# TravisWheelerLab/BATH

Hardware: AMD Instinct MI355X
Metric: DP Gcells/s + residues/s through bathsearch pipeline at 1/2/4/8 MI355X (higher is better)
Workload: dtype u8/i16 integer scores (SSV: exact binary16), f32 Forward

## Files before the change

### bath_amd/csrc/bath_kernels.hpp

```cpp
#pragma once
#include <climits>
#include <hip/hip_runtime.h>

#include <cstdint>

#include "bath_hip.h"

namespace bath {

typedef short s16x2 __attribute__((ext_vector_type(2)));

template <int CTRL, int ROW_MASK = 0xf>
__device__ __forceinline__ int dpp_i(int v, int old) { return __builtin_amdgcn_update_dpp(old, v, CTRL, ROW_MASK, 0xf, false); }
__device__ __forceinline__ int wave_shr1_i32(int v, int fill) { return dpp_i<0x138>(v, fill); }
__device__ __forceinline__ float wave_shr1_f32(float v, float fill) {
  return __builtin_bit_cast(float, __builtin_amdgcn_update_dpp(__builtin_bit_cast(int, fill), __builtin_bit_cast(int, v), 0x138, 0xf, 0xf, false));
}
__device__ __forceinline__ float wave_max_f32(float v) {
  const int ninf = (int)0xff800000;
#define BATH_FMAX_STEP(CTRL, MASK) v = fmaxf(v, __builtin_bit_cast(float, __builtin_amdgcn_update_dpp(ninf, __builtin_bit_cast(int, v), CTRL, MASK, 0xf, false)));
  BATH_FMAX_STEP(0x111, 0xf) BATH_FMAX_STEP(0x112, 0xf) BATH_FMAX_STEP(0x114, 0xf) BATH_FMAX_STEP(0x118, 0xf) BATH_FMAX_STEP(0x142, 0xa) BATH_FMAX_STEP(0x143, 0xc)
#undef BATH_FMAX_STEP
  return __builtin_bit_cast(float, __builtin_amdgcn_readlane(__builtin_bit_cast(int, v), 63));
}
__device__ __forceinline__ int wave_max_i32(int v) {
  v = max(v, dpp_i<0x111>(v, INT_MIN)); v = max(v, dpp_i<0x112>(v, INT_MIN)); v = max(v, dpp_i<0x114>(v, INT_MIN));
  v = max(v, dpp_i<0x118>(v, INT_MIN)); v = max(v, dpp_i<0x142, 0xa>(v, INT_MIN)); v = max(v, dpp_i<0x143, 0xc>(v, INT_MIN));
  return __builtin_amdgcn_readlane(v, 63);
}
__device__ __forceinline__ int wave_min_i32(int v) {
  v = min(v, dpp_i<0x111>(v, INT_MAX)); v = min(v, dpp_i<0x112>(v, INT_MAX)); v = min(v, dpp_i<0x114>(v, INT_MAX));
  v = min(v, dpp_i<0x118>(v, INT_MAX)); v = min(v, dpp_i<0x142, 0xa>(v, INT_MAX)); v = min(v, dpp_i<0x143, 0xc>(v, INT_MAX));
  return __builtin_amdgcn_readlane(v, 63);
}
__device__ __forceinline__ float wave_sum_f32(float v) {
#ifdef BATH_SUM_BPERMUTE
#pragma unroll
  for (int d = 32; d >= 1; d >>= 1) v += __shfl_xor(v, d, 64);
// ... 78 lines not shown
  return (grank == 0) ? kSsvBeginPair : far;
}
template <int G>
__device__ __forceinline__ int ssv_group_max(s16x2 xE) {
  typedef _Float16 h16x2 __attribute__((ext_vector_type(2)));
  const h16x2 h = __builtin_bit_cast(h16x2, xE);
  int v = (int)(fmaxf((float)h.x, (float)h.y) * 2048.0f) - 128;
#pragma unroll
  for (int d = SsvGroups<G>::TPW; d < 64; d <<= 1) v = max(v, __shfl_xor(v, d, 64));
  return v;
}

struct MsvConsts {
  int tbm, tec, base, bias;
  float scale_b;
};

__device__ __forceinline__ int ssv_classify(int v, int tjb, const MsvConsts &c, float *sc) {
  if (tjb + c.tbm + c.tec + c.bias >= 127) return BATH_ENORESULT;
  unsigned xE = (v >= -1 - c.bias) ? 255u : (unsigned)(v + 256);
  if ((int)xE >= 255 - c.bias) {
    *sc = INFINITY;
    return (c.base - tjb - c.tbm < 128) ? BATH_ENORESULT : BATH_ERANGE;
  }
  xE = (xE + (unsigned)(c.base - tjb - c.tbm) - 128u) & 0xffffu;
  if ((int)xE >= 255 - c.bias) { *sc = INFINITY; return BATH_ERANGE; }
  unsigned xJ = (xE - (unsigned)c.tec) & 0xffffu;
  if ((int)xJ > c.base) return BATH_ENORESULT;
  float r = ((float)((int)xJ - tjb) - (float)c.base);
  r /= c.scale_b;
  r = (float)((double)r - 3.0);
  *sc = r;
  return BATH_OK;
}

struct WindowRec { int32_t cand, n, k, length; float score; };

__device__ __forceinline__ float bias_forward(const uint8_t *s, int L, int M, const float *e , float p1) {
  const float L1 = (float)M / 8.0f;
  const float t00 = p1, t01 = 1.0f - p1, t10 = 1.0f / (L1 + 1.0f), t11 = L1 / (L1 + 1.0f);
  float logsc = 0.0f;
  if (L <= 0) return logsc;
  int x = min((int)s[0], 28);
  float d0 = e[2 * x] * 0.999f, d1 = e[2 * x + 1] * 0.001f;
  float mx = fmaxf(fmaxf(d0, 0.0f), d1);
  d0 /= mx; d1 /= mx;
  logsc += (float)log((double)mx);
  auto step = [&](int xx) {
    float n0 = 0.0f + d0 * t00; n0 = n0 + d1 * t10; n0 *= e[2 * xx];
    float n1 = 0.0f + d0 * t01; n1 = n1 + d1 * t11; n1 *= e[2 * xx + 1];
    mx = fmaxf(fmaxf(n0, 0.0f), n1);
    d0 = n0 / mx; d1 = n1 / mx;
    logsc += (float)log((double)mx);
  };
  int i = 1;
  uint32_t wnext = (i + 4 <= L) ? *reinterpret_cast<const uint32_t *>(s + i) : 0u;
  for (; i + 4 <= L; i += 4) {
    const uint32_t w = wnext;
    if (i + 8 <= L) wnext = *reinterpret_cast<const uint32_t *>(s + i + 4);
#pragma unroll
    for (int j = 0; j < 4; j++) step(min((int)((w >> (8 * j)) & 0xffu), 28));
  }
  for (; i < L; i++) step(min((int)s[i], 28));
  float end = 0.0f + d0 * 1.0f; end = end + d1 * 1.0f;
  logsc += (float)log((double)end);
  return logsc;
// ... 4 lines not shown
```

### bath_amd/csrc/bath_launch.hpp

```cpp
#pragma once
#include <utility>

#include "bath_common.hpp"

#define BATH_SSV_SHAPES(X)                                                                                   \
  X(16, 1) X(20, 1) X(24, 1) X(28, 1) X(32, 1) X(36, 1) X(40, 1) X(44, 1) X(48, 1) X(52, 1) X(56, 1) X(60, 1) X(64, 1)     \
  X(68, 1) X(72, 1) X(76, 1) X(80, 1) X(84, 1) X(88, 1) X(92, 1) X(96, 1) X(100, 1) X(104, 1) X(108, 1) X(112, 1)           \
  X(128, 1) X(144, 1) X(160, 1) X(176, 1) X(192, 1) X(208, 1)                                                \
  X(40, 2) X(48, 2) X(56, 2) X(64, 2) X(72, 2) X(76, 2)                                                     \
  X(112, 2) X(128, 2) X(144, 2) X(160, 2) X(176, 2) X(192, 2) X(208, 2)                                      \
  X(112, 4) X(128, 4) X(144, 4) X(160, 4) X(176, 4) X(192, 4) X(208, 4)                                      \
  X(112, 8) X(128, 8) X(144, 8) X(160, 8) X(176, 8) X(192, 8) X(208, 8)

namespace bath {

struct Cand {
  int64_t *window;  int32_t *sf;
  int32_t *startj;  int32_t *len;
  int16_t *v;
  int64_t *off;
  int32_t *msv_status, *vit_status, *fwd_status, *stage, *flags;
  float *usc, *nullsc, *filtersc, *vfsc, *fwdsc;
  double *P;
  int32_t *kminmax;
};

int build_orf_records(bath_hip_ctx *ctx, const Cand &cand, int nc, int64_t window_offset, bath_orf_result **d_out, int64_t *n_out);

struct VitWindowArgs {
  double invP_vit, invP_msv;
  const float *d_filtersc;
  const uint8_t *d_ssv_scores;
  void *d_wins;
  int *d_win_count;
  int win_cap;
  int32_t *d_kminmax;
};

int launch_ssv_lane(bath_hip_ctx *ctx, const bath_hip_oprofile *om, SeqView v, const int32_t *d_order, int16_t *d_v);
int launch_ssv_classify(bath_hip_ctx *ctx, const bath_hip_oprofile *om, int64_t n, const int32_t *d_len, const int16_t *d_v, float *d_sc, int32_t *d_status);
int launch_msv_wave(bath_hip_ctx *ctx, const bath_hip_oprofile *om, SeqView v, const int32_t *d_todo, int64_t ntodo, float *d_sc, int32_t *d_status, const int *ntodo_dev, bool lane_ok = true);
int launch_msv_lane(bath_hip_ctx *ctx, const bath_hip_oprofile *om, SeqView v, const int32_t *d_todo, int64_t ntodo, float *d_sc, int32_t *d_status, const int *ntodo_dev);
int launch_vit_wave(bath_hip_ctx *ctx, const bath_hip_oprofile *om, SeqView v, const int32_t *d_todo, int64_t ntodo, float *d_sc, int32_t *d_status,
                    const VitWindowArgs *wa, const int *ntodo_dev);
int launch_fwd_wave(bath_hip_ctx *ctx, const bath_hip_oprofile *om, SeqView v, const int32_t *d_todo, int64_t ntodo, float *d_sc, int32_t *d_status, const int *ntodo_dev,
                    float *d_xmx = nullptr, const int64_t *d_xmx_off = nullptr, float *d_dp = nullptr, const int64_t *d_dp_off = nullptr, int unihit = 0,
                    const int32_t *d_cfg_len = nullptr);
int launch_bwd_wave(bath_hip_ctx *ctx, const bath_hip_oprofile *om, SeqView v, int64_t n, const float *d_fwd_xmx, const int64_t *d_xmx_off,
                    float *d_sc, int32_t *d_status, float *d_bck_xmx, float *d_dp = nullptr, const int64_t *d_dp_off = nullptr, int unihit = 0);
int launch_bias_lane(bath_hip_ctx *ctx, const bath_hip_oprofile *om, SeqView v, const float *d_eo, int eo_stride, const int32_t *d_todo, int64_t ntodo,
                     float *d_nullsc, float *d_filtersc);

int vit_lane_supported(const bath_hip_oprofile *om);
int launch_len_sort(bath_hip_ctx *ctx, const int32_t *d_todo, const int *d_ntodo, const int32_t *d_len, int *d_bins, int32_t *d_sorted);
int launch_vit_lane(bath_hip_ctx *ctx, const bath_hip_oprofile *om, SeqView v, const int32_t *d_todo, int64_t ntodo, const int *ntodo_dev,
                    float *d_sc, int32_t *d_status, const VitWindowArgs *wa, const int *skip_dev = nullptr);
const int *len_sort_count_longer(const int *d_bins, int T);
int64_t lane_min_nt();
const char *vit_lane_kernel_name(const bath_hip_oprofile *om);
int launch_vit_sorted(bath_hip_ctx *ctx, const bath_hip_oprofile *om, SeqView v, const int32_t *d_todo, int64_t cap, const int *d_ntodo, const int32_t *d_len,
                      int *d_bins, int32_t *d_sorted, float *d_sc, int32_t *d_status, const VitWindowArgs *wa, const std::function<int(hipStream_t)> &beside);
struct MsvConsts;
MsvConsts msv_consts(const bath_hip_oprofile *om);

int pipeline_filters_survivors(bath_hip_ctx *ctx, const bath_hip_oprofile *om, const bath_hip_seqs *dna, const bath_pipeline_params *prm,
                               bath_pipeline_stats *stats, std::vector<PipelineSurvivor> *out, const uint8_t **d_pool);

struct FsWinDev {
  int64_t src_off;
  int64_t dst_off;
  int32_t seq_n, start, len, strand, kmin, kmax;
};
int fs_gather_view(bath_hip_ctx *ctx, const bath_hip_seqs *dna, std::vector<FsWinDev> &regs, const uint8_t *d_comp, bath_hip_seqs *view, const FsWinDev **d_desc_out);

struct WindowRec;
// ... 92 lines not shown
```

### bath_amd/csrc/bath_msv_lane.hip

```cpp
#include "bath_common.hpp"
#include "bath_kernels.hpp"
#include "bath_launch.hpp"

using namespace bath;

namespace bath {

__device__ __forceinline__ s16x2 msv_pkmax(s16x2 a, s16x2 b) {
  s16x2 r;
  asm("v_pk_max_f16 %0, %1, %2" : "=v"(r) : "v"(a), "v"(b));
  return r;
}

template <int NR>
__global__ __launch_bounds__(256, NR <= 76 ? 4 : 1) void msv_lane_kernel(SeqView sq, const int16_t *__restrict__ cost_tab , int row_bytes,
                                                                        const uint8_t *__restrict__ tjb_tab, MsvConsts c,
                                                                        const int32_t *__restrict__ todo, int64_t ntodo, const int *__restrict__ ntodo_dev,
                                                                        float *__restrict__ sc, int32_t *__restrict__ status) {
  extern __shared__ __attribute__((aligned(16))) char lds[];
  {
    const int n32 = kSsvRows * row_bytes / 4;
    const uint32_t *src = reinterpret_cast<const uint32_t *>(cost_tab);
    uint32_t *dst = reinterpret_cast<uint32_t *>(lds);
    for (int i = threadIdx.x; i < n32; i += blockDim.x) dst[i] = src[i];
  }
  __syncthreads();
  if (ntodo_dev) ntodo = *ntodo_dev;
  const int lane = threadIdx.x & 63;
  const int64_t nwaves = ((int64_t)gridDim.x * blockDim.x) >> 6;
  typedef _Float16 h16x2 __attribute__((ext_vector_type(2)));
  for (int64_t w = ((int64_t)blockIdx.x * blockDim.x + threadIdx.x) >> 6; w * 64 < ntodo; w += nwaves) {
    const int64_t job = w * 64 + lane;
    const bool live = job < ntodo;
    const int64_t sid = live ? (todo ? (int64_t)todo[job] : job) : 0;
    const int L = live ? sq.len[sid] : 0;
    const uint8_t *s = sq.data + sq.off[sid];
    const int Lw = wave_max_i32(L);
    const int tjb = tjb_tab[L];
    const int tjbm = (uint8_t)((int8_t)tjb + (int8_t)c.tbm);
    s16x2 reg[NR];
    const s16x2 zero = {0, 0};
#pragma unroll
    for (int r = 0; r < NR; r++) reg[r] = zero;
    int xJ = 0, xB = satu8(c.base - tjbm);
    bool overflow = false;
    uint2 res = make_uint2(0u, 0u);
    for (int i = 0; i < Lw; i++) {
      if ((i & 7) == 0) {
        if (i + 8 <= L) __builtin_memcpy(&res, s + i, 8);
        else {
          res = make_uint2(0u, 0u);
          for (int j = 0; j < 8 && i + j < L; j++) {
            const unsigned b = s[i + j];
            if (j < 4) res.x |= b << (8 * j); else res.y |= b << (8 * (j - 4));
          }
        }
      }
      const unsigned byte = (((i & 4) ? res.y : res.x) >> (8 * (i & 3))) & 0xffu;
      const int x = (i < L) ? min((int)byte, kKp - 1) : kRowReset;
      const ssv_i4 *row = reinterpret_cast<const ssv_i4 *>(lds + (size_t)x * row_bytes);
      const h16x2 bh = {(_Float16)((float)xB * (1.0f / 2048.0f)), (_Float16)((float)xB * (1.0f / 2048.0f))};
      const s16x2 xBv = __builtin_bit_cast(s16x2, bh);
      const s16x2 wrap = __builtin_bit_cast(s16x2, __builtin_amdgcn_alignbit(__builtin_bit_cast(unsigned, reg[NR - 1]), 0u, 16));
      s16x2 xE = zero, xE2 = zero;
#pragma unroll
      for (int g = NR / 4 - 1; g >= 0; g--) {
        const ssv_i4 inc = row[g];
        const int r = 4 * g;
        const s16x2 v3 = ssv_add(msv_pkmax(reg[r + 2], xBv), inc.w);
        const s16x2 v2 = ssv_add(msv_pkmax(reg[r + 1], xBv), inc.z);
        const s16x2 v1 = ssv_add(msv_pkmax(reg[r], xBv), inc.y);
        const s16x2 v0 = ssv_add(msv_pkmax((r > 0) ? reg[r - 1] : wrap, xBv), inc.x);
        reg[r + 3] = v3; reg[r + 2] = v2; reg[r + 1] = v1; reg[r] = v0;
        xE = ssv_max3(xE, v3, v2);
        xE2 = ssv_max3(xE2, v1, v0);
      }
      const h16x2 e1 = __builtin_bit_cast(h16x2, xE), e2 = __builtin_bit_cast(h16x2, xE2);
      int xEi = (int)(fmaxf(fmaxf((float)e1.x, (float)e1.y), fmaxf((float)e2.x, (float)e2.y)) * 2048.0f);
      if (xEi + c.bias >= 255) overflow = true;
      xEi = max(xEi - c.tec, 0);
      xJ = max(xJ, xEi);
      xB = max(max(c.base, xJ) - tjbm, 0);
    }
    if (live) {
      if (overflow) { sc[sid] = INFINITY; status[sid] = BATH_ERANGE; }
      else {
        float r = ((float)(xJ - tjb) - (float)c.base);
        r /= c.scale_b;
        r = (float)((double)r - 3.0);
        sc[sid] = r; status[sid] = BATH_OK;
      }
    }
  }
}

int launch_msv_lane(bath_hip_ctx *ctx, const bath_hip_oprofile *om, SeqView v, const int32_t *d_todo, int64_t ntodo, float *d_sc, int32_t *d_status, const int *ntodo_dev) {
  static const bool off = [] { const char *e = std::getenv("BATH_HIP_MSV_WAVE"); return e && e[0] == '1'; }();
  if (off || om->G != 1 || om->NR > 76 || !om->d_msv) return BATH_ENORESULT;
  if (ntodo == 0) return BATH_OK;
  const size_t shmem = (size_t)kSsvRows * om->ssv_row_bytes;
  const int64_t waves = (ntodo + 63) / 64;
  const int grid = (int)std::max<int64_t>(1, std::min<int64_t>((waves + 3) / 4, (int64_t)ctx->prop.multiProcessorCount * 4));
  bool launched = false;
#define BATH_MSV_CASE(N)                                                                                                               \
  if (!launched && om->NR == N) {                                                                                                      \
    hipLaunchKernelGGL((msv_lane_kernel<N>), dim3(grid), dim3(256), shmem, ctx->stream, v, om->d_msv, om->ssv_row_bytes, om->lt.d_tjb,   \
                       MsvConsts{om->tbm_b, om->tec_b, om->base_b, om->bias_b, om->scale_b}, d_todo, ntodo, ntodo_dev, d_sc, d_status); \
    launched = true;                                                                                                                   \
  }
  BATH_MSV_CASE(16) BATH_MSV_CASE(20) BATH_MSV_CASE(24) BATH_MSV_CASE(28) BATH_MSV_CASE(32) BATH_MSV_CASE(36) BATH_MSV_CASE(40) BATH_MSV_CASE(44)
  BATH_MSV_CASE(48) BATH_MSV_CASE(52) BATH_MSV_CASE(56) BATH_MSV_CASE(60) BATH_MSV_CASE(64) BATH_MSV_CASE(68) BATH_MSV_CASE(72) BATH_MSV_CASE(76)
#undef BATH_MSV_CASE
  if (!launched) return BATH_ENORESULT;
  BATH_HIP_TRY(ctx, hipGetLastError());
  return BATH_OK;
}

}
```

### bath_amd/csrc/bath_pipeline.hip

```cpp
#include <algorithm>
#include <cmath>
#include <cstring>
#include <cstdlib>
#include <map>
#include <thread>

#include "bath_common.hpp"
#include "bath_kernels.hpp"
#include "bath_launch.hpp"
#include "host_model.hpp"

using namespace bath;

namespace bath {

static const double kLog2 = 0.69314718055994529;

enum { FLAG_VIT_RUN = 1, FLAG_HAS_WIN = 2 };

struct Counters {
  int cand_count, todo_msv, todo_vit, todo_ssvb, todo_vit2, todo_fwd, win_count, overflow;
  int todo_lb, pad_;
  unsigned long long n_orfs, orf_res;
  unsigned long long n_past_msv, n_past_bias, n_past_vit, n_past_fwd;
// ... 77 lines not shown
        const int startj = (int32_t)(rec.aa_off - (2 * dna.off[w] + 96 * w + (int64_t)sf * orf_stream_pitch(dna.len[w])));
        const int C = dna.context[w], start_s = sf % 3 + 3 * startj + 1;
        if (sf < 3 ? (start_s + 3 * L - 1 < C) : (dna.len[w] - start_s + 1 < C)) r = (unsigned long long)L;
      }
      if (__ballot(r != 0)) { for (int d = 32; d >= 1; d >>= 1) r += __shfl_xor(r, d, 64); if (lane == 0) atomicAdd(&ctr->res_seen, r); }
    }
    if (live && grank == 0 && v >= (int)emit_thresh[min(L, thresh_max)]) {
      const int sf = (int)((unsigned)rec.len_sf >> 28);
      const int64_t w = rec.w;
      const int64_t stream = 2 * dna.off[w] + 96 * w + (int64_t)sf * orf_stream_pitch(dna.len[w]);
      const int startj = (int32_t)(rec.aa_off - stream);
      bool seen = false;
      if (dna.context) {
        const int C = dna.context[w], start_s = sf % 3 + 3 * startj + 1;
        seen = sf < 3 ? (start_s + 3 * L - 1 < C) : (dna.len[w] - start_s + 1 < C);
      }
      const int slot = seen ? cand_cap + 1 : atomicAdd(&ctr->cand_count, 1);
      if (seen) {
      } else if (slot < cand_cap) {
        cand.window[slot] = w; cand.sf[slot] = sf; cand.startj[slot] = startj; cand.len[slot] = L;
        cand.v[slot] = (int16_t)min(v, 32767); cand.off[slot] = rec.aa_off;
      } else atomicOr(&ctr->overflow, 1);
    }
  }
}

__device__ __forceinline__ double d_gumbel_surv(double x, double mu, double lambda) {
  const double ey = -exp(-lambda * (x - mu));
  if (fabs(ey) < 5e-9) return -ey;
  return 1.0 - exp(ey);
}
__device__ __forceinline__ double d_exp_surv(double x, double mu, double lambda) { return (x < mu) ? 1.0 : exp(-lambda * (x - mu)); }

__global__ void classify_kernel(Cand cand, int cand_cap, Counters *__restrict__ ctr, const uint8_t *__restrict__ tjb_tab, MsvConsts mc,
                                int32_t *__restrict__ todo_msv) {
  const int ncand = min(ctr->cand_count, cand_cap);
  for (int c = blockIdx.x * blockDim.x + threadIdx.x; c < ncand; c += gridDim.x * blockDim.x) {
    float sc = 0.f;
    const int st = ssv_classify(cand.v[c], tjb_tab[cand.len[c]], mc, &sc);
    cand.usc[c] = sc; cand.msv_status[c] = st; cand.stage[c] = 0; cand.flags[c] = 0;
    cand.vfsc[c] = -INFINITY; cand.fwdsc[c] = -INFINITY; cand.vit_status[c] = 0; cand.filtersc[c] = 0.f; cand.P[c] = 1.0;
    cand.kminmax[2 * c] = 1 << 30; cand.kminmax[2 * c + 1] = 0;
    if (st == BATH_ENORESULT) todo_msv[atomicAdd(&ctr->todo_msv, 1)] = c;
  }
}

__global__ void f1_bias_kernel(Cand cand, int cand_cap, Counters *__restrict__ ctr, Params p, const uint8_t *__restrict__ pool, int M,
                               const float *__restrict__ eo, const float *__restrict__ nullsc_tab, const float *__restrict__ p1_tab,
                               const float *__restrict__ lt1_tab, const float *__restrict__ lt2_tab,
                               int32_t *__restrict__ todo_vit, int32_t *__restrict__ todo_ssvb) {
  __shared__ float s_eo[kKp * 2];
  for (int i = threadIdx.x; i < kKp * 2; i += blockDim.x) s_eo[i] = eo[i];
  __syncthreads();
  const int ncand = min(ctr->cand_count, cand_cap);
  for (int c = blockIdx.x * blockDim.x + threadIdx.x; c < ncand; c += gridDim.x * blockDim.x) {
    const int L = cand.len[c];
    const float usc = cand.usc[c];
    const float nullsc = nullsc_tab[L];
    cand.nullsc[c] = nullsc;
    float seqsc = (float)((double)(usc - nullsc) / kLog2);
    double P = d_gumbel_surv(seqsc, p.evparam[0], p.evparam[1]);
    cand.P[c] = P;
    if (P > p.F1) continue;
    atomicAdd(&ctr->n_past_msv, 1ull); atomicAdd(&ctr->pos_past_msv, (unsigned long long)L * 3ull);
    cand.stage[c] = 1;
    float filtersc = nullsc;
    if (p.do_bias) {
      filtersc = bias_forward(pool + cand.off[c], L, M, s_eo, p1_tab[L]);
      filtersc = (filtersc + lt1_tab[L]) + lt2_tab[L];
      seqsc = (float)((double)(usc - filtersc) / kLog2);
      P = d_gumbel_surv(seqsc, p.evparam[0], p.evparam[1]);
      cand.P[c] = P; cand.filtersc[c] = filtersc;
      if (P > p.F1) continue;
    }
    cand.filtersc[c] = filtersc;
    atomicAdd(&ctr->n_past_bias, 1ull); atomicAdd(&ctr->pos_past_bias, (unsigned long long)L * 3ull);
    cand.stage[c] = 2;
    if (P > p.F2) { cand.flags[c] |= FLAG_VIT_RUN; todo_vit[atomicAdd(&ctr->todo_vit, 1)] = c; atomicAdd(&ctr->res_vit, (unsigned long long)L); }
    else todo_ssvb[atomicAdd(&ctr->todo_ssvb, 1)] = c;
  }
}

template <int C>
__global__ __launch_bounds__(256) void ssv_bath_kernel(Cand cand, const Counters *__restrict__ ctr, const int32_t *__restrict__ todo,
                                                       const uint8_t *__restrict__ pool, int M, const uint8_t *__restrict__ rb, int rb_stride,
                                                       const uint8_t *__restrict__ ssv_scores, const uint8_t *__restrict__ tjb_tab,
                                                       const float *__restrict__ nullsc_tab, MsvConsts mc, double invP_f1,
                                                       WindowRec *__restrict__ wins, int win_cap, Counters *__restrict__ ctrw) {
  const int lane = threadIdx.x & 63;
  const int64_t wid = ((int64_t)blockIdx.x * blockDim.x + threadIdx.x) >> 6;
  const int64_t nw = ((int64_t)gridDim.x * blockDim.x) >> 6;
  const int ntodo = ctr->todo_ssvb;
  const int Q = max(2, ((M - 1) / 16) + 1);
  for (int64_t job = wid; job < ntodo; job += nw) {
    const int c = todo[job];
    const int L = cand.len[c];
    const uint8_t *s = pool + cand.off[c];
    const int tjb = tjb_tab[L];
    const float nullsc = nullsc_tab[L];
    const int sc_thresh = (uint8_t)(int)ceil((((double)nullsc + ((double)(float)invP_f1 * kLog2) + 3.0) * (double)mc.scale_b) + mc.base + mc.tec + tjb);
    const int tjbm = (uint8_t)((int8_t)tjb + (int8_t)mc.tbm);
    const int xB = satu8(mc.base - tjbm);
    int kmin = 1 << 30, kmax = 0;
    int dp[C];
#pragma unroll
    for (int k = 0; k < C; k++) dp[k] = 0;
    const int ph = threadIdx.x & 63;
    int rbuf = (ph < L) ? (int)s[ph] : 0, rnext = 0;
    for (int i = 1; i <= L; i++) {
      const int j = (i - 1) & 63;
      if (j == 0) { const int q = i - 1 + 64 + ph; rnext = (q < L) ? (int)s[q] : 0; }
      const int x = min(__builtin_amdgcn_readlane(rbuf, j), kKp - 1);
      if (j == 63) rbuf = rnext;
// ... 444 lines not shown
    SeqView cv{W.pool, W.cand.off, W.cand.len, cap};

    int e = 0;
    BATH_HIP_TRY(ctx, hipEventRecord(ev[e++], ctx->stream));
    if ((st = launch_orf_scan(ctx, dna, tt, prm->min_orf_len, ob, &W.ctr->n_orfs, &W.ctr->orf_res, prm->strands)) != BATH_OK) return st;
    BATH_HIP_TRY(ctx, hipEventRecord(ev[e++], ctx->stream));
    {
      static const int ssv_chunk = [] { const char *e = std::getenv("BATH_HIP_SSV_CHUNK"); return e ? std::atoi(e) : 0; }();
      int blocks = ctx->prop.multiProcessorCount * 4;
      const int ssv_threads = 256;
      const int wpb = ssv_threads / 64;
      if (ssv_chunk > 0) blocks = (int)std::min<int64_t>((max_orfs + (int64_t)wpb * (64 / om->G) * ssv_chunk - 1) / ((int64_t)wpb * (64 / om->G) * ssv_chunk), 1 << 30);
      bool launched = false;
#define BATH_ORF_CASE(N, GG)                                                                                                     \
  if (!launched && NRk == N && om->G == GG) {                                                                                    \
    if (ssv_shmem > 64 * 1024) (void)bath::allow_max_lds((const void *)ssv_orf_kernel<N, GG>); \
    hipLaunchKernelGGL((ssv_orf_kernel<N, GG>), dim3(blocks), dim3(ssv_threads), ssv_shmem, ctx->stream, W.pool, ob.sorted, ob.ntotal,                  \
                       dna->view(), om->d_ssv, om->ssv_row_bytes, d_emit, max_orf, W.cand, W.cand_cap, W.ctr, ssv_chunk);        \
    launched = true;                                                                                                             \
  }
      BATH_SSV_SHAPES(BATH_ORF_CASE)
#undef BATH_ORF_CASE
      if (!launched) { ctx->set_error("SSV kernel: no tile shape for this model length"); return BATH_EINVAL; }
      BATH_HIP_TRY(ctx, hipGetLastError());
    }
    BATH_HIP_TRY(ctx, hipEventRecord(ev[e++], ctx->stream));
    hipStream_t bulk_stream = ctx->stream;
    struct StreamRestore { bath_hip_ctx *c; hipStream_t s; ~StreamRestore() { c->stream = s; } } stream_restore{ctx, bulk_stream};
    if (ctx->tail_stream) {
      BATH_HIP_TRY(ctx, hipStreamWaitEvent(ctx->tail_stream, ev[e - 1], 0));
      ctx->stream = ctx->tail_stream;
    }
    const bool few_cands = dna->total < lane_min_nt(), few_msv = dna->total < 2 * lane_min_nt();
    hipLaunchKernelGGL(classify_kernel, dim3(dec_blocks), dim3(256), 0, ctx->stream, W.cand, W.cand_cap, W.ctr, om->lt.d_tjb, mc, W.todo_msv);
    BATH_HIP_TRY(ctx, hipGetLastError());
    if ((st = launch_msv_wave(ctx, om, cv, W.todo_msv, cap, W.cand.usc, W.cand.msv_status, &W.ctr->todo_msv, !few_msv)) != BATH_OK) return st;
    BATH_HIP_TRY(ctx, hipEventRecord(ev[e++], ctx->stream));
    hipLaunchKernelGGL(f1_bias_kernel, dim3(dec_blocks), dim3(256), 0, ctx->stream, W.cand, W.cand_cap, W.ctr, P, W.pool, M, om->d_bias_eo,
                       om->lt.d_nullsc, om->lt.d_p1, om->lt.d_lt1, om->lt.d_lt2, W.todo_vit, W.todo_ssvb);
    BATH_HIP_TRY(ctx, hipGetLastError());
    BATH_HIP_TRY(ctx, hipEventRecord(ev[e++], ctx->stream));
    wa.d_filtersc = W.cand.filtersc; wa.d_ssv_scores = d_ssvsc; wa.d_wins = W.wins; wa.d_win_count = &W.ctr->win_count; wa.win_cap = W.win_cap;
    wa.d_kminmax = W.cand.kminmax;
    auto launch_ssvb = [&](hipStream_t stream) -> int {
      const int Cc = (M + 63) / 64;
      int Cs = -1;
      for (int opt : {1, 2, 3, 4, 6, 8, 12, 16, 24, 32, 52}) if (Cc <= opt) { Cs = opt; break; }
#define BATH_SSVB_CASE(N)                                                                                                          \
  case N:                                                                                                                          \
    hipLaunchKernelGGL(ssv_bath_kernel<N>, dim3(wave_grid_blocks(ctx) / 4), dim3(256), 0, stream, W.cand, W.ctr, W.todo_ssvb, W.pool, M,      \
                       om->d_rb, om->rb_stride, d_ssvsc, om->lt.d_tjb, om->lt.d_nullsc, mc, invP_f1, W.wins, W.win_cap, W.ctr);    \
    break;
      switch (Cs) {
        BATH_SSVB_CASE(1) BATH_SSVB_CASE(2) BATH_SSVB_CASE(3) BATH_SSVB_CASE(4) BATH_SSVB_CASE(6) BATH_SSVB_CASE(8)
        BATH_SSVB_CASE(12) BATH_SSVB_CASE(16) BATH_SSVB_CASE(24) BATH_SSVB_CASE(32) BATH_SSVB_CASE(52)
        default: ctx->set_error("model too long for the SSV window kernel"); return BATH_EINVAL;
      }
#undef BATH_SSVB_CASE
      return BATH_OK;
    };
    bool ssvb_done = false;
    if (vit_lane_supported(om) && !few_cands) {
      if ((st = launch_vit_sorted(ctx, om, cv, W.todo_vit, cap, &W.ctr->todo_vit, W.cand.len, W.len_bins, W.todo_sorted, W.cand.vfsc, W.cand.vit_status, &wa,
                                  launch_ssvb)) != BATH_OK) return st;
      ssvb_done = true;
    } else if ((st = launch_vit_wave(ctx, om, cv, W.todo_vit, cap, W.cand.vfsc, W.cand.vit_status, &wa, &W.ctr->todo_vit)) != BATH_OK) return st;
    BATH_HIP_TRY(ctx, hipEventRecord(ev[e++], ctx->stream));
    if (!ssvb_done && (st = launch_ssvb(ctx->stream)) != BATH_OK) return st;
    BATH_HIP_TRY(ctx, hipGetLastError());
    BATH_HIP_TRY(ctx, hipEventRecord(ev[e++], ctx->stream));
    hipLaunchKernelGGL(post_vit_kernel, dim3(dec_blocks), dim3(256), 0, ctx->stream, W.cand, W.cand_cap, W.ctr, P, W.todo_msv , W.todo_fwd);
    if (P.do_bias) {
      DevBuf &b_compo = ctx->scratch[36];
      BATH_HIP_TRY(ctx, b_compo.reserve((size_t)20 * 256 * 4 + (size_t)W.cand_cap * 20 * 4 + 256));
// ... 3 lines not shown
      hipLaunchKernelGGL(post_vit_local_kernel, dim3(std::max(1, dec_blocks)), dim3(64), 0, ctx->stream, W.cand, W.ctr, P, W.pool, M, d_bgf, d_compo,
                         om->lt.d_p1, om->lt.d_lt1, om->lt.d_lt2, W.todo_msv, W.todo_vit2, W.todo_fwd);
    }
    BATH_HIP_TRY(ctx, hipGetLastError());
    if ((st = launch_vit_wave(ctx, om, cv, W.todo_vit2, cap, W.cand.vfsc, W.cand.vit_status, nullptr, &W.ctr->todo_vit2)) != BATH_OK) return st;
    hipLaunchKernelGGL(post_vit2_kernel, dim3(64), dim3(256), 0, ctx->stream, W.cand, W.ctr, P, W.todo_vit2, W.todo_fwd);
    BATH_HIP_TRY(ctx, hipGetLastError());
    BATH_HIP_TRY(ctx, hipEventRecord(ev[e++], ctx->stream));
    ctx->fwd_rows_kept = nullptr; ctx->fwd_rows_off = nullptr;
    float *d_keep = nullptr; int64_t *d_keep_off = nullptr;
    if (ctx->keep_fwd_rows) {
      constexpr int64_t kKeepFloats = (int64_t)8 << 20;
      DevBuf &b_rows = ctx->scratch[38], &b_roff = ctx->scratch[39];
      BATH_HIP_TRY(ctx, b_rows.reserve((size_t)kKeepFloats * sizeof(float) + 64)); BATH_HIP_TRY(ctx, b_roff.reserve((size_t)cap * sizeof(int64_t) + 64));
      d_keep = b_rows.as<float>(); d_keep_off = b_roff.as<int64_t>();
      hipLaunchKernelGGL(fwd_keep_offsets_kernel, dim3(1), dim3(64), 0, ctx->stream, W.todo_fwd, &W.ctr->todo_fwd, W.cand.len, d_keep_off, kKeepFloats);
      BATH_HIP_TRY(ctx, hipGetLastError());
    }
    if ((st = launch_fwd_wave(ctx, om, cv, W.todo_fwd, cap, W.cand.fwdsc, W.cand.fwd_status, &W.ctr->todo_fwd, d_keep, d_keep_off)) != BATH_OK) return st;
    if (d_keep) { ctx->fwd_rows_kept = d_keep; ctx->fwd_rows_off = d_keep_off; }
    hipLaunchKernelGGL(final_kernel, dim3(dec_blocks), dim3(256), 0, ctx->stream, W.cand, W.ctr, P, W.todo_fwd);
    BATH_HIP_TRY(ctx, hipGetLastError());
    BATH_HIP_TRY(ctx, hipEventRecord(ev[e++], ctx->stream));

    BATH_HIP_TRY(ctx, hipMemcpyAsync(&hc, W.ctr, sizeof(Counters), hipMemcpyDeviceToHost, ctx->stream));
    BATH_HIP_TRY(ctx, hipStreamSynchronize(ctx->stream));
    if (hc.overflow || hc.cand_count > cap || hc.win_count > W.win_cap) {
      if (attempt >= 4) { ctx->set_error("candidate / window buffers overflowed repeatedly"); return BATH_EMEM; }
      if (hc.overflow || hc.cand_count > cap) cap = std::max<int64_t>(cap * 2, (int64_t)hc.cand_count + 1024);
      if (hc.win_count > W.win_cap) win_need = hc.win_count + hc.win_count / 4 + 1024;
      continue;
    }
    static const char *names[] = {"translate_orfs", "ssv_f1", "classify_msv", "f1_bias", "viterbi_windows", "ssv_windows", "post_vit", "forward_final"};
    static const int64_t launches[] = {4, 1, 2, 1, 4, 1, 3, 2};
    ctx->timings.clear();
    for (int i = 0; i + 1 < e; i++) {
      float ms = 0.f;
      BATH_HIP_TRY(ctx, hipEventElapsedTime(&ms, ev[i], ev[i + 1]));
      ctx->timings.push_back(StageTiming{names[i], ms, launches[i]});
    }
    break;
  }

  if (stats) {
    stats->nres = nres; stats->n_orfs = (int64_t)hc.n_orfs;
    stats->n_past_msv = (int64_t)hc.n_past_msv; stats->n_past_bias = (int64_t)hc.n_past_bias;
    stats->n_past_vit = (int64_t)hc.n_past_vit; stats->n_past_fwd = (int64_t)hc.n_past_fwd;
    stats->pos_past_msv = (int64_t)hc.pos_past_msv; stats->pos_past_bias = (int64_t)hc.pos_past_bias;
    stats->pos_past_vit = (int64_t)hc.pos_past_vit; stats->pos_past_fwd = (int64_t)hc.pos_past_fwd;
    stats->cells_msv = (int64_t)(hc.orf_res - hc.res_seen) * M; stats->cells_vit = (int64_t)hc.res_vit * M; stats->cells_fwd = (int64_t)hc.res_fwd * M;
  }

  if (results) {
    bath_orf_result *d_rec = nullptr;
    int64_t nrec = 0;
    if (dna->n > (int64_t)UINT32_MAX || dna->maxlen / 3 >= (1 << 28)) { ctx->set_error("block too large for the ORF records' sort key (2^32 windows, 805 Mnt per window)"); return BATH_ERANGE; }
    if ((st = build_orf_records(ctx, W.cand, hc.cand_count, dna->is_part ? dna->first_window : 0, &d_rec, &nrec)) != BATH_OK) return st;
    ctx->d_records = d_rec; ctx->n_records = nrec;
    if (!dna->is_part) {
      BATH_HIP_TRY(ctx, ctx->results_pinned.reserve((size_t)std::max<int64_t>(nrec, 1) * sizeof(bath_orf_result)));
      if (nrec > 0) BATH_HIP_TRY(ctx, hipMemcpyAsync(ctx->results_pinned.p, d_rec, (size_t)nrec * sizeof(bath_orf_result), hipMemcpyDeviceToHost, ctx->stream));
      BATH_HIP_TRY(ctx, hipStreamSynchronize(ctx->stream));
      *results = ctx->results_pinned.as<bath_orf_result>();
    } else *results = nullptr;
    if (n_results) *n_results = nrec;
  } else if (n_results) *n_results = (int64_t)hc.n_past_msv;
  if (state) { state->W = W; state->hc = hc; state->d_ssvsc = d_ssvsc; state->d_bgf = d_bgf; state->tt = tt; }
// ... 622 lines not shown
```

Baseline: 197.6 billion.

## Fuse classify, MSV rescoring and F1 bias filter into one stage kernel

Adds a fused msv_stage_kernel. Each thread classifies its candidate, rescores it with the per-lane MSV DP when SSV gave no result, and then runs the F1/bias filter in the same launch. This drops two kernel launches and the todo_msv indirection. In exchange, every block copies the cost table into LDS, and lanes whose candidate needs no rescore sit idle while the rest of the wave runs the MSV loop, so the wave runs as long as its longest rescore. It also launches over cand_cap blocks rather than a bounded grid, which may leave many blocks that exit immediately.

```diff
diff --git a/bath_amd/csrc/bath_kernels.hpp b/bath_amd/csrc/bath_kernels.hpp
--- a/bath_amd/csrc/bath_kernels.hpp
+++ b/bath_amd/csrc/bath_kernels.hpp
@@ -4,6 +4,7 @@
 
 #include <cstdint>
 
+#include "bath_common.hpp"
 #include "bath_hip.h"
 
 namespace bath {
@@ -148,6 +149,67 @@
   r = (float)((double)r - 3.0);
   *sc = r;
   return BATH_OK;
+}
+
+__device__ __forceinline__ s16x2 msv_pkmax(s16x2 a, s16x2 b) {
+  s16x2 r;
+  asm("v_pk_max_f16 %0, %1, %2" : "=v"(r) : "v"(a), "v"(b));
+  return r;
+}
+template <int NR>
+__device__ __forceinline__ int msv_lane_rows(const char *lds, int row_bytes, const uint8_t *s, int L, int Lw, int tjbm, const MsvConsts &c, bool *overflow) {
+  typedef _Float16 h16x2 __attribute__((ext_vector_type(2)));
+  s16x2 reg[NR];
+  const s16x2 zero = {0, 0};
+#pragma unroll
+  for (int r = 0; r < NR; r++) reg[r] = zero;
+  int xJ = 0, xB = satu8(c.base - tjbm);
+  bool over = false;
+  uint2 res = make_uint2(0u, 0u);
+  for (int i = 0; i < Lw; i++) {
+    if ((i & 7) == 0) {
+      if (i + 8 <= L) __builtin_memcpy(&res, s + i, 8);
+      else {
+        res = make_uint2(0u, 0u);
+        for (int j = 0; j < 8 && i + j < L; j++) {
+          const unsigned b = s[i + j];
+          if (j < 4) res.x |= b << (8 * j); else res.y |= b << (8 * (j - 4));
+        }
+      }
+    }
+    const unsigned byte = (((i & 4) ? res.y : res.x) >> (8 * (i & 3))) & 0xffu;
+    const int x = (i < L) ? min((int)byte, kKp - 1) : kRowReset;
+    const ssv_i4 *row = reinterpret_cast<const ssv_i4 *>(lds + (size_t)x * row_bytes);
+    const h16x2 bh = {(_Float16)((float)xB * (1.0f / 2048.0f)), (_Float16)((float)xB * (1.0f / 2048.0f))};
+    const s16x2 xBv = __builtin_bit_cast(s16x2, bh);
+    const s16x2 wrap = __builtin_bit_cast(s16x2, __builtin_amdgcn_alignbit(__builtin_bit_cast(unsigned, reg[NR - 1]), 0u, 16));
+    s16x2 xE = zero, xE2 = zero;
+#pragma unroll
+    for (int g = NR / 4 - 1; g >= 0; g--) {
+      const ssv_i4 inc = row[g];
+      const int r = 4 * g;
+      const s16x2 v3 = ssv_add(msv_pkmax(reg[r + 2], xBv), inc.w);
+      const s16x2 v2 = ssv_add(msv_pkmax(reg[r + 1], xBv), inc.z);
+      const s16x2 v1 = ssv_add(msv_pkmax(reg[r], xBv), inc.y);
+      const s16x2 v0 = ssv_add(msv_pkmax((r > 0) ? reg[r - 1] : wrap, xBv), inc.x);
+      reg[r + 3] = v3; reg[r + 2] = v2; reg[r + 1] = v1; reg[r] = v0;
+      xE = ssv_max3(xE, v3, v2);
+      xE2 = ssv_max3(xE2, v1, v0);
+    }
+    const h16x2 e1 = __builtin_bit_cast(h16x2, xE), e2 = __builtin_bit_cast(h16x2, xE2);
+    int xEi = (int)(fmaxf(fmaxf((float)e1.x, (float)e1.y), fmaxf((float)e2.x, (float)e2.y)) * 2048.0f);
+    if (xEi + c.bias >= 255) over = true;
+    xEi = max(xEi - c.tec, 0);
+    xJ = max(xJ, xEi);
+    xB = max(max(c.base, xJ) - tjbm, 0);
+  }
+  *overflow = over;
+  return xJ;
+}
+__device__ __forceinline__ float msv_lane_score(int xJ, int tjb, const MsvConsts &c) {
+  float r = ((float)(xJ - tjb) - (float)c.base);
+  r /= c.scale_b;
+  return (float)((double)r - 3.0);
 }
 
 struct WindowRec { int32_t cand, n, k, length; float score; };
diff --git a/bath_amd/csrc/bath_launch.hpp b/bath_amd/csrc/bath_launch.hpp
--- a/bath_amd/csrc/bath_launch.hpp
+++ b/bath_amd/csrc/bath_launch.hpp
@@ -41,6 +41,7 @@
 int launch_ssv_classify(bath_hip_ctx *ctx, const bath_hip_oprofile *om, int64_t n, const int32_t *d_len, const int16_t *d_v, float *d_sc, int32_t *d_status);
 int launch_msv_wave(bath_hip_ctx *ctx, const bath_hip_oprofile *om, SeqView v, const int32_t *d_todo, int64_t ntodo, float *d_sc, int32_t *d_status, const int *ntodo_dev, bool lane_ok = true);
 int launch_msv_lane(bath_hip_ctx *ctx, const bath_hip_oprofile *om, SeqView v, const int32_t *d_todo, int64_t ntodo, float *d_sc, int32_t *d_status, const int *ntodo_dev);
+bool msv_stage_supported(const bath_hip_oprofile *om);
 int launch_vit_wave(bath_hip_ctx *ctx, const bath_hip_oprofile *om, SeqView v, const int32_t *d_todo, int64_t ntodo, float *d_sc, int32_t *d_status,
                     const VitWindowArgs *wa, const int *ntodo_dev);
 int launch_fwd_wave(bath_hip_ctx *ctx, const bath_hip_oprofile *om, SeqView v, const int32_t *d_todo, int64_t ntodo, float *d_sc, int32_t *d_status, const int *ntodo_dev,
diff --git a/bath_amd/csrc/bath_msv_lane.hip b/bath_amd/csrc/bath_msv_lane.hip
--- a/bath_amd/csrc/bath_msv_lane.hip
+++ b/bath_amd/csrc/bath_msv_lane.hip
@@ -5,12 +5,6 @@
 using namespace bath;
 
 namespace bath {
-
-__device__ __forceinline__ s16x2 msv_pkmax(s16x2 a, s16x2 b) {
-  s16x2 r;
-  asm("v_pk_max_f16 %0, %1, %2" : "=v"(r) : "v"(a), "v"(b));
-  return r;
-}
 
 template <int NR>
 __global__ __launch_bounds__(256, NR <= 76 ? 4 : 1) void msv_lane_kernel(SeqView sq, const int16_t *__restrict__ cost_tab , int row_bytes,
@@ -28,7 +22,6 @@
   if (ntodo_dev) ntodo = *ntodo_dev;
   const int lane = threadIdx.x & 63;
   const int64_t nwaves = ((int64_t)gridDim.x * blockDim.x) >> 6;
-  typedef _Float16 h16x2 __attribute__((ext_vector_type(2)));
   for (int64_t w = ((int64_t)blockIdx.x * blockDim.x + threadIdx.x) >> 6; w * 64 < ntodo; w += nwaves) {
     const int64_t job = w * 64 + lane;
     const bool live = job < ntodo;
@@ -38,65 +31,23 @@
     const int Lw = wave_max_i32(L);
     const int tjb = tjb_tab[L];
     const int tjbm = (uint8_t)((int8_t)tjb + (int8_t)c.tbm);
-    s16x2 reg[NR];
-    const s16x2 zero = {0, 0};
-#pragma unroll
-    for (int r = 0; r < NR; r++) reg[r] = zero;
-    int xJ = 0, xB = satu8(c.base - tjbm);
     bool overflow = false;
-    uint2 res = make_uint2(0u, 0u);
-    for (int i = 0; i < Lw; i++) {
-      if ((i & 7) == 0) {
-        if (i + 8 <= L) __builtin_memcpy(&res, s + i, 8);
-        else {
-          res = make_uint2(0u, 0u);
-          for (int j = 0; j < 8 && i + j < L; j++) {
-            const unsigned b = s[i + j];
-            if (j < 4) res.x |= b << (8 * j); else res.y |= b << (8 * (j - 4));
-          }
-        }
-      }
-      const unsigned byte = (((i & 4) ? res.y : res.x) >> (8 * (i & 3))) & 0xffu;
-      const int x = (i < L) ? min((int)byte, kKp - 1) : kRowReset;
-      const ssv_i4 *row = reinterpret_cast<const ssv_i4 *>(lds + (size_t)x * row_bytes);
-      const h16x2 bh = {(_Float16)((float)xB * (1.0f / 2048.0f)), (_Float16)((float)xB * (1.0f / 2048.0f))};
-      const s16x2 xBv = __builtin_bit_cast(s16x2, bh);
-      const s16x2 wrap = __builtin_bit_cast(s16x2, __builtin_amdgcn_alignbit(__builtin_bit_cast(unsigned, reg[NR - 1]), 0u, 16));
-      s16x2 xE = zero, xE2 = zero;
-#pragma unroll
-      for (int g = NR / 4 - 1; g >= 0; g--) {
-        const ssv_i4 inc = row[g];
-        const int r = 4 * g;
-        const s16x2 v3 = ssv_add(msv_pkmax(reg[r + 2], xBv), inc.w);
-        const s16x2 v2 = ssv_add(msv_pkmax(reg[r + 1], xBv), inc.z);
-        const s16x2 v1 = ssv_add(msv_pkmax(reg[r], xBv), inc.y);
-        const s16x2 v0 = ssv_add(msv_pkmax((r > 0) ? reg[r - 1] : wrap, xBv), inc.x);
-        reg[r + 3] = v3; reg[r + 2] = v2; reg[r + 1] = v1; reg[r] = v0;
-        xE = ssv_max3(xE, v3, v2);
-        xE2 = ssv_max3(xE2, v1, v0);
-      }
-      const h16x2 e1 = __builtin_bit_cast(h16x2, xE), e2 = __builtin_bit_cast(h16x2, xE2);
-      int xEi = (int)(fmaxf(fmaxf((float)e1.x, (float)e1.y), fmaxf((float)e2.x, (float)e2.y)) * 2048.0f);
-      if (xEi + c.bias >= 255) overflow = true;
-      xEi = max(xEi - c.tec, 0);
-      xJ = max(xJ, xEi);
-      xB = max(max(c.base, xJ) - tjbm, 0);
-    }
+    const int xJ = msv_lane_rows<NR>(lds, row_bytes, s, L, Lw, tjbm, c, &overflow);
     if (live) {
       if (overflow) { sc[sid] = INFINITY; status[sid] = BATH_ERANGE; }
-      else {
-        float r = ((float)(xJ - tjb) - (float)c.base);
-        r /= c.scale_b;
-        r = (float)((double)r - 3.0);
-        sc[sid] = r; status[sid] = BATH_OK;
-      }
+      else { sc[sid] = msv_lane_score(xJ, tjb, c); status[sid] = BATH_OK; }
     }
   }
 }
 
+bool msv_stage_supported(const bath_hip_oprofile *om) {
+  static const bool off = [] { const char *e = std::getenv("BATH_HIP_MSV_WAVE"); return e && e[0] == '1'; }();
+  if (off || om->G != 1 || om->NR > 76 || !om->d_msv) return false;
+  return true;
+}
+
 int launch_msv_lane(bath_hip_ctx *ctx, const bath_hip_oprofile *om, SeqView v, const int32_t *d_todo, int64_t ntodo, float *d_sc, int32_t *d_status, const int *ntodo_dev) {
-  static const bool off = [] { const char *e = std::getenv("BATH_HIP_MSV_WAVE"); return e && e[0] == '1'; }();
-  if (off || om->G != 1 || om->NR > 76 || !om->d_msv) return BATH_ENORESULT;
+  if (!msv_stage_supported(om)) return BATH_ENORESULT;
   if (ntodo == 0) return BATH_OK;
   const size_t shmem = (size_t)kSsvRows * om->ssv_row_bytes;
   const int64_t waves = (ntodo + 63) / 64;
diff --git a/bath_amd/csrc/bath_pipeline.hip b/bath_amd/csrc/bath_pipeline.hip
--- a/bath_amd/csrc/bath_pipeline.hip
+++ b/bath_amd/csrc/bath_pipeline.hip
@@ -133,53 +133,94 @@
 }
 __device__ __forceinline__ double d_exp_surv(double x, double mu, double lambda) { return (x < mu) ? 1.0 : exp(-lambda * (x - mu)); }
 
+__device__ __forceinline__ int cand_classify(const Cand &cand, int c, int tjb, const MsvConsts &mc) {
+  float sc = 0.f;
+  const int st = ssv_classify(cand.v[c], tjb, mc, &sc);
+  cand.usc[c] = sc; cand.msv_status[c] = st; cand.stage[c] = 0; cand.flags[c] = 0;
+  cand.vfsc[c] = -INFINITY; cand.fwdsc[c] = -INFINITY; cand.vit_status[c] = 0; cand.filtersc[c] = 0.f; cand.P[c] = 1.0;
+  cand.kminmax[2 * c] = 1 << 30; cand.kminmax[2 * c + 1] = 0;
+  return st;
+}
+
 __global__ void classify_kernel(Cand cand, int cand_cap, Counters *__restrict__ ctr, const uint8_t *__restrict__ tjb_tab, MsvConsts mc,
                                 int32_t *__restrict__ todo_msv) {
   const int ncand = min(ctr->cand_count, cand_cap);
   for (int c = blockIdx.x * blockDim.x + threadIdx.x; c < ncand; c += gridDim.x * blockDim.x) {
-    float sc = 0.f;
-    const int st = ssv_classify(cand.v[c], tjb_tab[cand.len[c]], mc, &sc);
-    cand.usc[c] = sc; cand.msv_status[c] = st; cand.stage[c] = 0; cand.flags[c] = 0;
-    cand.vfsc[c] = -INFINITY; cand.fwdsc[c] = -INFINITY; cand.vit_status[c] = 0; cand.filtersc[c] = 0.f; cand.P[c] = 1.0;
-    cand.kminmax[2 * c] = 1 << 30; cand.kminmax[2 * c + 1] = 0;
-    if (st == BATH_ENORESULT) todo_msv[atomicAdd(&ctr->todo_msv, 1)] = c;
-  }
-}
-
-__global__ void f1_bias_kernel(Cand cand, int cand_cap, Counters *__restrict__ ctr, Params p, const uint8_t *__restrict__ pool, int M,
-                               const float *__restrict__ eo, const float *__restrict__ nullsc_tab, const float *__restrict__ p1_tab,
-                               const float *__restrict__ lt1_tab, const float *__restrict__ lt2_tab,
+    if (cand_classify(cand, c, tjb_tab[cand.len[c]], mc) == BATH_ENORESULT) todo_msv[atomicAdd(&ctr->todo_msv, 1)] = c;
+  }
+}
+
+struct F1Tables { const float *eo, *nullsc, *p1, *lt1, *lt2; };
+__device__ __forceinline__ void cand_f1_bias(const Cand &cand, int c, Counters *__restrict__ ctr, const Params &p, const uint8_t *__restrict__ pool, int M,
+                                             const float *s_eo , const F1Tables &t,
+                                             int32_t *__restrict__ todo_vit, int32_t *__restrict__ todo_ssvb) {
+  const int L = cand.len[c];
+  const float usc = cand.usc[c];
+  const float nullsc = t.nullsc[L];
+  cand.nullsc[c] = nullsc;
+  float seqsc = (float)((double)(usc - nullsc) / kLog2);
+  double P = d_gumbel_surv(seqsc, p.evparam[0], p.evparam[1]);
+  cand.P[c] = P;
+  if (P > p.F1) return;
+  atomicAdd(&ctr->n_past_msv, 1ull); atomicAdd(&ctr->pos_past_msv, (unsigned long long)L * 3ull);
+  cand.stage[c] = 1;
+  float filtersc = nullsc;
+  if (p.do_bias) {
+    filtersc = bias_forward(pool + cand.off[c], L, M, s_eo, t.p1[L]);
+    filtersc = (filtersc + t.lt1[L]) + t.lt2[L];
+    seqsc = (float)((double)(usc - filtersc) / kLog2);
+    P = d_gumbel_surv(seqsc, p.evparam[0], p.evparam[1]);
+    cand.P[c] = P; cand.filtersc[c] = filtersc;
+    if (P > p.F1) return;
+  }
+  cand.filtersc[c] = filtersc;
+  atomicAdd(&ctr->n_past_bias, 1ull); atomicAdd(&ctr->pos_past_bias, (unsigned long long)L * 3ull);
+  cand.stage[c] = 2;
+  if (P > p.F2) { cand.flags[c] |= FLAG_VIT_RUN; todo_vit[atomicAdd(&ctr->todo_vit, 1)] = c; atomicAdd(&ctr->res_vit, (unsigned long long)L); }
+  else todo_ssvb[atomicAdd(&ctr->todo_ssvb, 1)] = c;
+}
+
+__global__ void f1_bias_kernel(Cand cand, int cand_cap, Counters *__restrict__ ctr, Params p, const uint8_t *__restrict__ pool, int M, F1Tables t,
                                int32_t *__restrict__ todo_vit, int32_t *__restrict__ todo_ssvb) {
   __shared__ float s_eo[kKp * 2];
-  for (int i = threadIdx.x; i < kKp * 2; i += blockDim.x) s_eo[i] = eo[i];
+  for (int i = threadIdx.x; i < kKp * 2; i += blockDim.x) s_eo[i] = t.eo[i];
   __syncthreads();
   const int ncand = min(ctr->cand_count, cand_cap);
-  for (int c = blockIdx.x * blockDim.x + threadIdx.x; c < ncand; c += gridDim.x * blockDim.x) {
-    const int L = cand.len[c];
-    const float usc = cand.usc[c];
-    const float nullsc = nullsc_tab[L];
-    cand.nullsc[c] = nullsc;
-    float seqsc = (float)((double)(usc - nullsc) / kLog2);
-    double P = d_gumbel_surv(seqsc, p.evparam[0], p.evparam[1]);
-    cand.P[c] = P;
-    if (P > p.F1) continue;
-    atomicAdd(&ctr->n_past_msv, 1ull); atomicAdd(&ctr->pos_past_msv, (unsigned long long)L * 3ull);
-    cand.stage[c] = 1;
-    float filtersc = nullsc;
-    if (p.do_bias) {
-      filtersc = bias_forward(pool + cand.off[c], L, M, s_eo, p1_tab[L]);
-      filtersc = (filtersc + lt1_tab[L]) + lt2_tab[L];
-      seqsc = (float)((double)(usc - filtersc) / kLog2);
-      P = d_gumbel_surv(seqsc, p.evparam[0], p.evparam[1]);
-      cand.P[c] = P; cand.filtersc[c] = filtersc;
-      if (P > p.F1) continue;
-    }
-    cand.filtersc[c] = filtersc;
-    atomicAdd(&ctr->n_past_bias, 1ull); atomicAdd(&ctr->pos_past_bias, (unsigned long long)L * 3ull);
-    cand.stage[c] = 2;
-    if (P > p.F2) { cand.flags[c] |= FLAG_VIT_RUN; todo_vit[atomicAdd(&ctr->todo_vit, 1)] = c; atomicAdd(&ctr->res_vit, (unsigned long long)L); }
-    else todo_ssvb[atomicAdd(&ctr->todo_ssvb, 1)] = c;
-  }
+  for (int c = blockIdx.x * blockDim.x + threadIdx.x; c < ncand; c += gridDim.x * blockDim.x) cand_f1_bias(cand, c, ctr, p, pool, M, s_eo, t, todo_vit, todo_ssvb);
+}
+
+template <int NR>
+__global__ __launch_bounds__(256, 4) void msv_stage_kernel(Cand cand, int cand_cap, Counters *__restrict__ ctr,
+                                                           const int16_t *__restrict__ cost_tab , int row_bytes,
+                                                           const uint8_t *__restrict__ tjb_tab, MsvConsts mc, Params p, const uint8_t *__restrict__ pool, int M,
+                                                           F1Tables t, int32_t *__restrict__ todo_vit, int32_t *__restrict__ todo_ssvb) {
+  extern __shared__ __attribute__((aligned(16))) char lds[];
+  __shared__ float s_eo[kKp * 2];
+  const int ncand = min(ctr->cand_count, cand_cap);
+  if ((int64_t)blockIdx.x * blockDim.x >= ncand) return;
+  {
+    const int n32 = kSsvRows * row_bytes / 4;
+    const uint32_t *src = reinterpret_cast<const uint32_t *>(cost_tab);
+    uint32_t *dst = reinterpret_cast<uint32_t *>(lds);
+    for (int i = threadIdx.x; i < n32; i += blockDim.x) dst[i] = src[i];
+    for (int i = threadIdx.x; i < kKp * 2; i += blockDim.x) s_eo[i] = t.eo[i];
+  }
+  __syncthreads();
+  const int64_t job = (int64_t)blockIdx.x * blockDim.x + threadIdx.x;
+  const bool live = job < ncand;
+  const int c = live ? (int)job : 0;
+  const int L = live ? cand.len[c] : 0;
+  const int tjb = tjb_tab[L];
+  const bool rescore = live && cand_classify(cand, c, tjb, mc) == BATH_ENORESULT;
+  const int Lr = rescore ? L : 0;
+  const uint8_t *s = pool + (rescore ? cand.off[c] : 0);
+  bool overflow = false;
+  const int xJ = msv_lane_rows<NR>(lds, row_bytes, s, Lr, wave_max_i32(Lr), (uint8_t)((int8_t)tjb + (int8_t)mc.tbm), mc, &overflow);
+  if (rescore) {
+    if (overflow) { cand.usc[c] = INFINITY; cand.msv_status[c] = BATH_ERANGE; }
+    else { cand.usc[c] = msv_lane_score(xJ, tjb, mc); cand.msv_status[c] = BATH_OK; }
+  }
+  if (live) cand_f1_bias(cand, c, ctr, p, pool, M, s_eo, t, todo_vit, todo_ssvb);
 }
 
 template <int C>
@@ -690,14 +731,33 @@
       ctx->stream = ctx->tail_stream;
     }
     const bool few_cands = dna->total < lane_min_nt(), few_msv = dna->total < 2 * lane_min_nt();
-    hipLaunchKernelGGL(classify_kernel, dim3(dec_blocks), dim3(256), 0, ctx->stream, W.cand, W.cand_cap, W.ctr, om->lt.d_tjb, mc, W.todo_msv);
-    BATH_HIP_TRY(ctx, hipGetLastError());
-    if ((st = launch_msv_wave(ctx, om, cv, W.todo_msv, cap, W.cand.usc, W.cand.msv_status, &W.ctr->todo_msv, !few_msv)) != BATH_OK) return st;
-    BATH_HIP_TRY(ctx, hipEventRecord(ev[e++], ctx->stream));
-    hipLaunchKernelGGL(f1_bias_kernel, dim3(dec_blocks), dim3(256), 0, ctx->stream, W.cand, W.cand_cap, W.ctr, P, W.pool, M, om->d_bias_eo,
-                       om->lt.d_nullsc, om->lt.d_p1, om->lt.d_lt1, om->lt.d_lt2, W.todo_vit, W.todo_ssvb);
-    BATH_HIP_TRY(ctx, hipGetLastError());
-    BATH_HIP_TRY(ctx, hipEventRecord(ev[e++], ctx->stream));
+    const F1Tables f1t{om->d_bias_eo, om->lt.d_nullsc, om->lt.d_p1, om->lt.d_lt1, om->lt.d_lt2};
+    const bool msv_stage = !few_msv && msv_stage_supported(om);
+    if (msv_stage) {
+      bool launched = false;
+#define BATH_MSV_STAGE_CASE(N)                                                                                                              \
+  if (!launched && NRk == N) {                                                                                                              \
+    hipLaunchKernelGGL((msv_stage_kernel<N>), dim3((unsigned)((W.cand_cap + 255) / 256)), dim3(256), ssv_shmem, ctx->stream, W.cand, W.cand_cap, W.ctr, om->d_msv, \
+                       om->ssv_row_bytes, om->lt.d_tjb, mc, P, W.pool, M, f1t, W.todo_vit, W.todo_ssvb);                                      \
+    launched = true;                                                                                                                        \
+  }
+      BATH_MSV_STAGE_CASE(16) BATH_MSV_STAGE_CASE(20) BATH_MSV_STAGE_CASE(24) BATH_MSV_STAGE_CASE(28) BATH_MSV_STAGE_CASE(32) BATH_MSV_STAGE_CASE(36)
+      BATH_MSV_STAGE_CASE(40) BATH_MSV_STAGE_CASE(44) BATH_MSV_STAGE_CASE(48) BATH_MSV_STAGE_CASE(52) BATH_MSV_STAGE_CASE(56) BATH_MSV_STAGE_CASE(60)
+      BATH_MSV_STAGE_CASE(64) BATH_MSV_STAGE_CASE(68) BATH_MSV_STAGE_CASE(72) BATH_MSV_STAGE_CASE(76)
+#undef BATH_MSV_STAGE_CASE
+      if (!launched) { ctx->set_error("MSV stage kernel: no tile shape for this model length"); return BATH_EINVAL; }
+      BATH_HIP_TRY(ctx, hipGetLastError());
+      BATH_HIP_TRY(ctx, hipEventRecord(ev[e++], ctx->stream));
+      BATH_HIP_TRY(ctx, hipEventRecord(ev[e++], ctx->stream));
+    } else {
+      hipLaunchKernelGGL(classify_kernel, dim3(dec_blocks), dim3(256), 0, ctx->stream, W.cand, W.cand_cap, W.ctr, om->lt.d_tjb, mc, W.todo_msv);
+      BATH_HIP_TRY(ctx, hipGetLastError());
+      if ((st = launch_msv_wave(ctx, om, cv, W.todo_msv, cap, W.cand.usc, W.cand.msv_status, &W.ctr->todo_msv, !few_msv)) != BATH_OK) return st;
+      BATH_HIP_TRY(ctx, hipEventRecord(ev[e++], ctx->stream));
+      hipLaunchKernelGGL(f1_bias_kernel, dim3(dec_blocks), dim3(256), 0, ctx->stream, W.cand, W.cand_cap, W.ctr, P, W.pool, M, f1t, W.todo_vit, W.todo_ssvb);
+      BATH_HIP_TRY(ctx, hipGetLastError());
+      BATH_HIP_TRY(ctx, hipEventRecord(ev[e++], ctx->stream));
+    }
     wa.d_filtersc = W.cand.filtersc; wa.d_ssv_scores = d_ssvsc; wa.d_wins = W.wins; wa.d_win_count = &W.ctr->win_count; wa.win_cap = W.win_cap;
     wa.d_kminmax = W.cand.kminmax;
     auto launch_ssvb = [&](hipStream_t stream) -> int {
@@ -767,7 +827,7 @@
       continue;
     }
     static const char *names[] = {"translate_orfs", "ssv_f1", "classify_msv", "f1_bias", "viterbi_windows", "ssv_windows", "post_vit", "forward_final"};
-    static const int64_t launches[] = {4, 1, 2, 1, 4, 1, 3, 2};
+    const int64_t launches[] = {4, 1, msv_stage ? 1 : 2, msv_stage ? 0 : 1, 4, 1, 3, 2};
     ctx->timings.clear();
     for (int i = 0; i + 1 < e; i++) {
       float ms = 0.f;
```

New measurement: 202.5 billion, median of 6. +2.5%, better.
